# collabora/WhisperLive

Hardware: NVIDIA H100
Metric: audio-sec/sec (RTF^-1) Whisper large-v3, 32 streams, beam 4 (higher is better)
Workload: dtype f16

## Files before the change

### whisperlive_b200/csrc/common.cuh

```cuda
#pragma once
#include <cuda.h>
#include <cuda_fp16.h>
#include <cuda_runtime.h>
#include <stdint.h>
#include <stdio.h>
#include <string.h>
#include <string>
#include <utility>

#define WL_OK 0
#define WL_ERR_CUDA -1
#define WL_ERR_ARG -2
#define WL_ERR_STATE -3
#define WL_ERR_NOMEM -4

namespace wl {

struct Error {
  int code;
  std::string msg;
};

#define WL_CUDA(expr)                                                                         \
  do {                                                                                        \
    cudaError_t _e = (expr);                                                                  \
    if (_e != cudaSuccess) {                                                                  \
      char _b[512];                                                                           \
      snprintf(_b, sizeof(_b), "%s:%d: %s -> %s", __FILE__, __LINE__, #expr, cudaGetErrorString(_e)); \
      throw wl::Error{WL_ERR_CUDA, _b};                                                       \
    }                                                                                         \
  } while (0)

#define WL_CHECK(cond, code, ...)                                  \
  do {                                                             \
    if (!(cond)) {                                                 \
      char _b[512];                                                \
      snprintf(_b, sizeof(_b), __VA_ARGS__);                       \
      throw wl::Error{code, std::string(_b)};                      \
    }                                                              \
  } while (0)

static inline int cdiv(long a, long b) { return (int)((a + b - 1) / b); }
void note_launch(int n);

bool pdl_active();
struct PdlScope {
  explicit PdlScope(bool on);
  ~PdlScope();
  bool prev;
};

#ifdef __CUDACC__
template <typename... KArgs, typename... Args>
static inline void launch_kernel(void (*kernel)(KArgs...), dim3 grid, dim3 block, size_t smem, cudaStream_t st, Args&&... args) {
  cudaLaunchConfig_t cfg;
  memset(&cfg, 0, sizeof(cfg));
  cfg.gridDim = grid;
  cfg.blockDim = block;
  cfg.dynamicSmemBytes = smem;
  cfg.stream = st;
  cudaLaunchAttribute attr[1];
  attr[0].id = cudaLaunchAttributeProgrammaticStreamSerialization;
  attr[0].val.programmaticStreamSerializationAllowed = 1;
  cfg.attrs = attr;
  cfg.numAttrs = pdl_active() ? 1 : 0;
  WL_CUDA(cudaLaunchKernelEx(&cfg, kernel, KArgs(std::forward<Args>(args))...));
}

constexpr unsigned TL_CAP = 1u << 20;
static __device__ unsigned long long* wl_tl_buf = nullptr;
#ifndef WLB200_TL
#define WLB200_TL 0
#endif
__device__ __forceinline__ void tl_stamp_any(int kernel_id, int what) {
  if (!WLB200_TL) return;
  unsigned long long* buf = wl_tl_buf;
  if (buf != nullptr) {
    unsigned long long t;
    asm volatile("mov.u64 %0, %%globaltimer;" : "=l"(t));
    const unsigned idx = atomicAdd(reinterpret_cast<unsigned*>(buf), 1u);
    if (idx < TL_CAP) buf[1 + idx] = (t << 8) | ((unsigned long long)kernel_id << 2) | (unsigned long long)what;
  }
}
__device__ __forceinline__ void tl_stamp(int kernel_id, int what) {
  if (blockIdx.x == 0 && blockIdx.y == 0 && threadIdx.x == 0) tl_stamp_any(kernel_id, what);
}
static inline void tl_bind_tu(unsigned long long* p) { cudaMemcpyToSymbol(wl_tl_buf, &p, sizeof(p)); }
enum TlKernel : int { TL_EMBED = 1, TL_LN = 2, TL_GEMM_PART = 3, TL_SELF = 4, TL_CROSS = 5, TL_COMBINE = 6, TL_GELU = 7,
                      TL_SROWS = 8, TL_SSTREAMS = 9, TL_GEMM = 10, TL_DSTEP = 11 };

__device__ __forceinline__ uint32_t smem_u32(const void* p) { return (uint32_t)__cvta_generic_to_shared(p); }
__device__ __forceinline__ int lane_id() { return threadIdx.x & 31; }

__device__ __forceinline__ bool elect_one() {
  uint32_t pred;
  asm volatile(
      "{\n\t.reg .pred p;\n\t.reg .b32 r;\n\t"
      "elect.sync r|p, 0xffffffff;\n\t"
      "selp.u32 %0, 1, 0, p;\n\t}"
      : "=r"(pred));
  return pred != 0;
}

__device__ __forceinline__ float gelu_erf(float x) {
  const float ax = fabsf(x);
  float t, e;
  asm("rcp.approx.ftz.f32 %0, %1;" : "=f"(t) : "f"(fmaf(0.3275911f * 0.70710678118654752440f, ax, 1.0f)));
  const float w = ax * 0.84932180028801904272f;
  asm("ex2.approx.ftz.f32 %0, %1;" : "=f"(e) : "f"(-w * w));
  float poly = fmaf(0.5f * 1.061405429f, t, 0.5f * -1.453152027f);
  poly = fmaf(poly, t, 0.5f * 1.421413741f);
  poly = fmaf(poly, t, 0.5f * -0.284496736f);
  poly = fmaf(poly, t, 0.5f * 0.254829592f);
  return fmaxf(x, 0.f) - ax * (poly * t * e);
}

__device__ __forceinline__ void pdl_wait() { asm volatile("griddepcontrol.wait;" ::: "memory"); }
__device__ __forceinline__ void pdl_trigger() { asm volatile("griddepcontrol.launch_dependents;" ::: "memory"); }

__device__ __forceinline__ void named_bar_sync(int id, int n) { asm volatile("bar.sync %0, %1;" ::"r"(id), "r"(n) : "memory"); }
__device__ __forceinline__ void named_bar_arrive(int id, int n) { asm volatile("bar.arrive %0, %1;" ::"r"(id), "r"(n) : "memory"); }

template <int R>
__device__ __forceinline__ void setmaxnreg_dec() { asm volatile("setmaxnreg.dec.sync.aligned.u32 %0;" ::"n"(R)); }
template <int R>
__device__ __forceinline__ void setmaxnreg_inc() { asm volatile("setmaxnreg.inc.sync.aligned.u32 %0;" ::"n"(R)); }

__device__ __forceinline__ float warp_sum(float v) {
#pragma unroll
  for (int o = 16; o > 0; o >>= 1) v += __shfl_xor_sync(0xffffffffu, v, o);
  return v;
}
__device__ __forceinline__ float warp_max(float v) {
#pragma unroll
  for (int o = 16; o > 0; o >>= 1) v = fmaxf(v, __shfl_xor_sync(0xffffffffu, v, o));
  return v;
}

__device__ __forceinline__ void mbar_init(uint64_t* bar, uint32_t count) {
  asm volatile("mbarrier.init.shared::cta.b64 [%0], %1;" ::"r"(smem_u32(bar)), "r"(count));
}
__device__ __forceinline__ void mbar_fence_init() { asm volatile("fence.mbarrier_init.release.cluster;" ::: "memory"); }
__device__ __forceinline__ void mbar_expect_tx(uint64_t* bar, uint32_t bytes) {
  asm volatile("mbarrier.arrive.expect_tx.shared::cta.b64 _, [%0], %1;" ::"r"(smem_u32(bar)), "r"(bytes) : "memory");
}
__device__ __forceinline__ void mbar_arrive(uint64_t* bar) {
  asm volatile("mbarrier.arrive.shared::cta.b64 _, [%0];" ::"r"(smem_u32(bar)) : "memory");
}
__device__ __forceinline__ void mbar_wait(uint64_t* bar, uint32_t parity) {
  asm volatile(
      "{\n\t.reg .pred p;\n\t"
      "WAIT_%=:\n\t"
      "mbarrier.try_wait.parity.shared::cta.b64 p, [%0], %1;\n\t"
      "@p bra DONE_%=;\n\t"
      "bra WAIT_%=;\n\t"
      "DONE_%=:\n\t}" ::"r"(smem_u32(bar)),
      "r"(parity)
      : "memory");
}
__device__ __forceinline__ void fence_proxy_async() { asm volatile("fence.proxy.async.shared::cta;" ::: "memory"); }

__device__ __forceinline__ void tma_prefetch_desc(const void* tmap) {
  asm volatile("prefetch.tensormap [%0];" ::"l"(tmap) : "memory");
}
__device__ __forceinline__ void tma_load_4d(void* dst, const void* tmap, uint64_t* bar, int c0, int c1, int c2, int c3) {
  asm volatile(
      "cp.async.bulk.tensor.4d.shared::cluster.global.tile.mbarrier::complete_tx::bytes [%0], [%1, {%3, %4, %5, %6}], [%2];" ::
          "r"(smem_u32(dst)),
      "l"(tmap), "r"(smem_u32(bar)), "r"(c0), "r"(c1), "r"(c2), "r"(c3)
      : "memory");
}
__device__ __forceinline__ void bulk_load_1d(void* dst, const void* src, uint32_t bytes, uint64_t* bar) {
  asm volatile("cp.async.bulk.shared::cluster.global.mbarrier::complete_tx::bytes [%0], [%1], %2, [%3];" ::"r"(
                   smem_u32(dst)),
               "l"(src), "r"(bytes), "r"(smem_u32(bar))
               : "memory");
}

__device__ __forceinline__ void wgmma_fence() { asm volatile("wgmma.fence.sync.aligned;" ::: "memory"); }
__device__ __forceinline__ void wgmma_commit() { asm volatile("wgmma.commit_group.sync.aligned;" ::: "memory"); }
template <int N>
__device__ __forceinline__ void wgmma_wait() { asm volatile("wgmma.wait_group.sync.aligned %0;" ::"n"(N) : "memory"); }
template <int R>
__device__ __forceinline__ void wgmma_fence_regs(float (&d)[R]) {
#pragma unroll
  for (int i = 0; i < R; ++i) asm volatile("" : "+f"(d[i])::"memory");
}

template <int N>
__device__ __forceinline__ void wgmma_ss(float (&d)[N / 2], uint64_t da, uint64_t db, uint32_t scale_d);
template <>
__device__ __forceinline__ void wgmma_ss<16>(float (&d)[8], uint64_t da, uint64_t db, uint32_t scale_d) {
  asm volatile(
      "{\n\t.reg .pred p;\n\tsetp.ne.b32 p, %10, 0;\n\t"
      "wgmma.mma_async.sync.aligned.m64n16k16.f32.f16.f16 {"
      "%0, %1, %2, %3, %4, %5, %6, %7"
      "}, %8, %9, p, 1, 1, 0, 0;\n\t}"
      : "+f"(d[0]), "+f"(d[1]), "+f"(d[2]), "+f"(d[3]), "+f"(d[4]), "+f"(d[5]), "+f"(d[6]), "+f"(d[7])
      : "l"(da), "l"(db), "r"(scale_d));
}

template <>
__device__ __forceinline__ void wgmma_ss<32>(float (&d)[16], uint64_t da, uint64_t db, uint32_t scale_d) {
  asm volatile(
      "{\n\t.reg .pred p;\n\tsetp.ne.b32 p, %18, 0;\n\t"
      "wgmma.mma_async.sync.aligned.m64n32k16.f32.f16.f16 {"
      "%0, %1, %2, %3, %4, %5, %6, %7, %8, %9, %10, %11, %12, %13, %14, %15"
      "}, %16, %17, p, 1, 1, 0, 0;\n\t}"
      : "+f"(d[0]), "+f"(d[1]), "+f"(d[2]), "+f"(d[3]), "+f"(d[4]), "+f"(d[5]), "+f"(d[6]), "+f"(d[7]),
        "+f"(d[8]), "+f"(d[9]), "+f"(d[10]), "+f"(d[11]), "+f"(d[12]), "+f"(d[13]), "+f"(d[14]), "+f"(d[15])
      : "l"(da), "l"(db), "r"(scale_d));
}

template <>
__device__ __forceinline__ void wgmma_ss<64>(float (&d)[32], uint64_t da, uint64_t db, uint32_t scale_d) {
  asm volatile(
      "{\n\t.reg .pred p;\n\tsetp.ne.b32 p, %34, 0;\n\t"
      "wgmma.mma_async.sync.aligned.m64n64k16.f32.f16.f16 {"
      "%0, %1, %2, %3, %4, %5, %6, %7, %8, %9, %10, %11, %12, %13, %14, %15,"
      "%16, %17, %18, %19, %20, %21, %22, %23, %24, %25, %26, %27, %28, %29, %30, %31"
      "}, %32, %33, p, 1, 1, 0, 0;\n\t}"
      : "+f"(d[0]), "+f"(d[1]), "+f"(d[2]), "+f"(d[3]), "+f"(d[4]), "+f"(d[5]), "+f"(d[6]), "+f"(d[7]),
        "+f"(d[8]), "+f"(d[9]), "+f"(d[10]), "+f"(d[11]), "+f"(d[12]), "+f"(d[13]), "+f"(d[14]), "+f"(d[15]),
        "+f"(d[16]), "+f"(d[17]), "+f"(d[18]), "+f"(d[19]), "+f"(d[20]), "+f"(d[21]), "+f"(d[22]), "+f"(d[23]),
        "+f"(d[24]), "+f"(d[25]), "+f"(d[26]), "+f"(d[27]), "+f"(d[28]), "+f"(d[29]), "+f"(d[30]), "+f"(d[31])
      : "l"(da), "l"(db), "r"(scale_d));
}

template <>
__device__ __forceinline__ void wgmma_ss<128>(float (&d)[64], uint64_t da, uint64_t db, uint32_t scale_d) {
  asm volatile(
      "{\n\t.reg .pred p;\n\tsetp.ne.b32 p, %66, 0;\n\t"
      "wgmma.mma_async.sync.aligned.m64n128k16.f32.f16.f16 {"
      "%0, %1, %2, %3, %4, %5, %6, %7, %8, %9, %10, %11, %12, %13, %14, %15,"
      "%16, %17, %18, %19, %20, %21, %22, %23, %24, %25, %26, %27, %28, %29, %30, %31,"
      "%32, %33, %34, %35, %36, %37, %38, %39, %40, %41, %42, %43, %44, %45, %46, %47,"
      "%48, %49, %50, %51, %52, %53, %54, %55, %56, %57, %58, %59, %60, %61, %62, %63"
      "}, %64, %65, p, 1, 1, 0, 0;\n\t}"
      : "+f"(d[0]), "+f"(d[1]), "+f"(d[2]), "+f"(d[3]), "+f"(d[4]), "+f"(d[5]), "+f"(d[6]), "+f"(d[7]),
        "+f"(d[8]), "+f"(d[9]), "+f"(d[10]), "+f"(d[11]), "+f"(d[12]), "+f"(d[13]), "+f"(d[14]), "+f"(d[15]),
        "+f"(d[16]), "+f"(d[17]), "+f"(d[18]), "+f"(d[19]), "+f"(d[20]), "+f"(d[21]), "+f"(d[22]), "+f"(d[23]),
        "+f"(d[24]), "+f"(d[25]), "+f"(d[26]), "+f"(d[27]), "+f"(d[28]), "+f"(d[29]), "+f"(d[30]), "+f"(d[31]),
        "+f"(d[32]), "+f"(d[33]), "+f"(d[34]), "+f"(d[35]), "+f"(d[36]), "+f"(d[37]), "+f"(d[38]), "+f"(d[39]),
        "+f"(d[40]), "+f"(d[41]), "+f"(d[42]), "+f"(d[43]), "+f"(d[44]), "+f"(d[45]), "+f"(d[46]), "+f"(d[47]),
        "+f"(d[48]), "+f"(d[49]), "+f"(d[50]), "+f"(d[51]), "+f"(d[52]), "+f"(d[53]), "+f"(d[54]), "+f"(d[55]),
        "+f"(d[56]), "+f"(d[57]), "+f"(d[58]), "+f"(d[59]), "+f"(d[60]), "+f"(d[61]), "+f"(d[62]), "+f"(d[63])
      : "l"(da), "l"(db), "r"(scale_d));
}

__device__ __forceinline__ void wgmma_rs_n64(float (&d)[32], const uint32_t (&a)[4], uint64_t db, uint32_t scale_d) {
  asm volatile(
      "{\n\t.reg .pred p;\n\tsetp.ne.b32 p, %37, 0;\n\t"
      "wgmma.mma_async.sync.aligned.m64n64k16.f32.f16.f16 {"
      "%0, %1, %2, %3, %4, %5, %6, %7, %8, %9, %10, %11, %12, %13, %14, %15,"
      "%16, %17, %18, %19, %20, %21, %22, %23, %24, %25, %26, %27, %28, %29, %30, %31"
      "}, {%32, %33, %34, %35}, %36, p, 1, 1, 0;\n\t}"
      : "+f"(d[0]), "+f"(d[1]), "+f"(d[2]), "+f"(d[3]), "+f"(d[4]), "+f"(d[5]), "+f"(d[6]), "+f"(d[7]),
        "+f"(d[8]), "+f"(d[9]), "+f"(d[10]), "+f"(d[11]), "+f"(d[12]), "+f"(d[13]), "+f"(d[14]), "+f"(d[15]),
        "+f"(d[16]), "+f"(d[17]), "+f"(d[18]), "+f"(d[19]), "+f"(d[20]), "+f"(d[21]), "+f"(d[22]), "+f"(d[23]),
        "+f"(d[24]), "+f"(d[25]), "+f"(d[26]), "+f"(d[27]), "+f"(d[28]), "+f"(d[29]), "+f"(d[30]), "+f"(d[31])
      : "r"(a[0]), "r"(a[1]), "r"(a[2]), "r"(a[3]), "l"(db), "r"(scale_d));
}

__device__ __forceinline__ uint64_t wgmma_desc_sw128(uint32_t smem_addr) {
  uint64_t d = 0;
  d |= (uint64_t)((smem_addr & 0x3FFFFu) >> 4);
  d |= (uint64_t)1 << 16;
  d |= (uint64_t)(1024 >> 4) << 32;
  d |= (uint64_t)1 << 62;
  return d;
}

template <int BN>
__device__ __forceinline__ void wgmma_tile_k64(float (&acc)[BN / 2], const uint8_t* sa, const uint8_t* sb, int wg, bool accumulate) {
  const uint64_t adesc = wgmma_desc_sw128(smem_u32(sa + wg * 64 * 128));
  const uint64_t bdesc = wgmma_desc_sw128(smem_u32(sb));
#pragma unroll
  for (int k = 0; k < 4; ++k) wgmma_ss<BN>(acc, adesc + (uint64_t)(2 * k), bdesc + (uint64_t)(2 * k), (accumulate || k > 0) ? 1u : 0u);
}

template <int R, class F>
__device__ __forceinline__ void wgmma_acc_foreach(const float (&d)[R], F&& f) {
  const int l = threadIdx.x & 31, w = (threadIdx.x >> 5) & 3;
  const int r0 = 16 * w + (l >> 2), c0 = 2 * (l & 3);
#pragma unroll
  for (int c = 0; c < R / 4; ++c)
#pragma unroll
    for (int i = 0; i < 2; ++i)
#pragma unroll
      for (int j = 0; j < 2; ++j) f(r0 + 8 * i, 8 * c + c0 + j, d[4 * c + 2 * i + j]);
}
#endif

}
```

### whisperlive_b200/csrc/gemm.cu

```cuda
#include "gemm.cuh"

#include <algorithm>
#include <atomic>
#include <cstdlib>
#include <cstring>
#include <map>
#include <mutex>
#include <vector>

namespace wl {

static std::atomic<long> g_gemm_launches{0};
long gemm_launch_count() { return g_gemm_launches.load(); }

struct GemmKParams {
  int M, N, K;
  int zn1;
  int a_batched, b_batched;
  int a_pos[3], b_pos[3];
  GemmEpilogue e;
  int vec_ok;
  int nz;
  int n_fastest;
};

constexpr int BM = 128;
constexpr int BK = 64;
constexpr int A_STAGE_BYTES = BM * BK * 2;

enum EpiKind : int { EPI_ROW = 0, EPI_COL = 1, EPI_HEADSPLIT = 2 };

template <int cnt, int KIND>
__device__ __forceinline__ void epilogue_chunk(const GemmKParams& p, long m, int n0, const uint32_t (&v)[cnt], int i1, int i2) {
  const GemmEpilogue& e = p.e;
  if (m >= p.M) return;
  if constexpr (KIND == EPI_HEADSPLIT && cnt >= 8) {
    const int mi = (int)m;
    const int b = mi / e.hs_S, s = mi % e.hs_S;
    const int h = n0 >> 6, dd = n0 & 63;
    const long slot = e.hs_slots[b];
    float x[cnt];
#pragma unroll
    for (int i = 0; i < cnt; ++i) x[i] = __uint_as_float(v[i]);
    if (e.bias) {
#pragma unroll
      for (int i = 0; i < cnt; i += 8) {
        if (n0 + i >= p.N) break;
#pragma unroll
        for (int j = 0; j < 8; ++j) x[i + j] += e.bias[n0 + i + j];
      }
    }
    __half* dst = (__half*)e.out + slot * e.hs_slot_stride + ((long)h * e.hs_S + s) * 64;
#pragma unroll
    for (int i = 0; i < cnt; i += 8) {
      if (n0 + i >= p.N) break;
      __align__(16) __half2 h2[4];
#pragma unroll
      for (int j = 0; j < 4; ++j) h2[j] = __floats2half2_rn(x[i + 2 * j], x[i + 2 * j + 1]);
      *reinterpret_cast<uint4*>(dst + ((((dd + i) >> 3) ^ (s & 7)) << 3)) = *reinterpret_cast<const uint4*>(h2);
    }
    return;
  }
  const long obase = (long)i1 * e.ob1 + (long)i2 * e.ob2 + m * e.ldm;
  const long rbase = (long)i1 * e.rb1 + (long)i2 * e.rb2 + m * e.rldm;
  const float bm = (e.bias && e.bias_on_m) ? e.bias[m] : 0.f;
  if constexpr (KIND == EPI_ROW && cnt >= 8) {
    if (n0 + cnt <= p.N) {
      float x[cnt];
#pragma unroll
      for (int i = 0; i < cnt; ++i) x[i] = __uint_as_float(v[i]) + bm;
      if (e.bias && !e.bias_on_m) {
#pragma unroll
        for (int i = 0; i < cnt; i += 4) {
          const float4 b4 = *reinterpret_cast<const float4*>(e.bias + n0 + i);
          x[i] += b4.x; x[i + 1] += b4.y; x[i + 2] += b4.z; x[i + 3] += b4.w;
        }
      }
      if (e.gelu) {
#pragma unroll
        for (int i = 0; i < cnt; ++i) x[i] = gelu_erf(x[i]);
      }
      if (e.resid) {
        const float* r = e.resid + rbase + n0;
        float4 r4[cnt / 4];
#pragma unroll
        for (int i = 0; i < cnt / 4; ++i) r4[i] = *reinterpret_cast<const float4*>(r + 4 * i);
#pragma unroll
        for (int i = 0; i < cnt / 4; ++i) {
          x[4 * i] += r4[i].x; x[4 * i + 1] += r4[i].y; x[4 * i + 2] += r4[i].z; x[4 * i + 3] += r4[i].w;
        }
      }
#pragma unroll
      for (int i = 0; i < cnt; i += 8) {
        if (e.out_f32) {
          float* o = (float*)e.out + obase + n0 + i;
          *reinterpret_cast<float4*>(o) = make_float4(x[i], x[i + 1], x[i + 2], x[i + 3]);
          *reinterpret_cast<float4*>(o + 4) = make_float4(x[i + 4], x[i + 5], x[i + 6], x[i + 7]);
        } else {
          __align__(16) __half2 h2[4];
#pragma unroll
          for (int j = 0; j < 4; ++j) h2[j] = __floats2half2_rn(x[i + 2 * j], x[i + 2 * j + 1]);
          *reinterpret_cast<uint4*>((__half*)e.out + obase + n0 + i) = *reinterpret_cast<const uint4*>(h2);
        }
      }
      return;
    }
#pragma unroll
    for (int i = 0; i < cnt; i += 8) {
      const int n = n0 + i;
      if (n >= p.N) break;
      if (n + 8 > p.N) {
#pragma unroll
        for (int j = 0; j < 8; ++j) {
          if (n + j < p.N) {
            float x1 = __uint_as_float(v[i + j]) + bm;
            if (e.bias && !e.bias_on_m) x1 += e.bias[n + j];
            if (e.gelu) x1 = gelu_erf(x1);
            if (e.resid) x1 += e.resid[rbase + n + j];
            if (e.out_f32) ((float*)e.out)[obase + n + j] = x1;
            else ((__half*)e.out)[obase + n + j] = __float2half_rn(x1);
          }
        }
        continue;
      }
      float x[8];
#pragma unroll
      for (int j = 0; j < 8; ++j) x[j] = __uint_as_float(v[i + j]) + bm;
      if (e.bias && !e.bias_on_m) {
        const float4 b0 = *reinterpret_cast<const float4*>(e.bias + n), b1 = *reinterpret_cast<const float4*>(e.bias + n + 4);
        x[0] += b0.x; x[1] += b0.y; x[2] += b0.z; x[3] += b0.w;
        x[4] += b1.x; x[5] += b1.y; x[6] += b1.z; x[7] += b1.w;
      }
      if (e.gelu) {
#pragma unroll
        for (int j = 0; j < 8; ++j) x[j] = gelu_erf(x[j]);
      }
      if (e.resid) {
        const float* r = e.resid + rbase + n;
        const float4 r0 = *reinterpret_cast<const float4*>(r), r1 = *reinterpret_cast<const float4*>(r + 4);
        x[0] += r0.x; x[1] += r0.y; x[2] += r0.z; x[3] += r0.w;
        x[4] += r1.x; x[5] += r1.y; x[6] += r1.z; x[7] += r1.w;
      }
      if (e.out_f32) {
        float* o = (float*)e.out + obase + n;
        *reinterpret_cast<float4*>(o) = make_float4(x[0], x[1], x[2], x[3]);
        *reinterpret_cast<float4*>(o + 4) = make_float4(x[4], x[5], x[6], x[7]);
      } else {
        __align__(16) __half2 h2[4];
#pragma unroll
        for (int j = 0; j < 4; ++j) h2[j] = __floats2half2_rn(x[2 * j], x[2 * j + 1]);
        *reinterpret_cast<uint4*>((__half*)e.out + obase + n) = *reinterpret_cast<const uint4*>(h2);
      }
    }
    return;
  }
  if constexpr (KIND == EPI_COL || cnt < 8) {
#pragma unroll
  for (int i = 0; i < cnt; ++i) {
    const int n = n0 + i;
    if (n >= p.N) break;
    float x = __uint_as_float(v[i]) + bm;
    if (e.bias && !e.bias_on_m) x += e.bias[n];
    if (e.gelu) x = gelu_erf(x);
    if (e.resid) x += e.resid[rbase + (long)n * e.rldn];
    const long o = obase + (long)n * e.ldn;
    if (e.out_f32) ((float*)e.out)[o] = x;
    else ((__half*)e.out)[o] = __float2half_rn(x);
  }
  }
}

__device__ __forceinline__ void tile_decode(const GemmKParams& p, int t, int tiles_m, int tiles_n, int& tile_m, int& tile_n, int& zz) {
  if (p.n_fastest) {
    tile_n = t % tiles_n;
    const int r = t / tiles_n;
    tile_m = r % tiles_m;
    zz = r / tiles_m;
  } else {
    tile_m = t % tiles_m;
    const int r = t / tiles_m;
    tile_n = r % tiles_n;
    zz = r / tiles_n;
  }
}

template <int BN>
struct EpiStage {
  static constexpr int CH = BN < 64 ? BN : 64;
  static constexpr int LD = CH + 4;
  static constexpr int BYTES = 2 * 64 * LD * 4;
};
template <int BN, int STAGES>
__host__ __device__ constexpr int gemm_smem_bytes() { return STAGES * (A_STAGE_BYTES + BN * BK * 2) + EpiStage<BN>::BYTES + 1024 + 512; }

struct TileCoord {
  int tile_m, tile_n, i1, i2;
};
__device__ __forceinline__ TileCoord tile_coord(const GemmKParams& p, int t, int tiles_m, int tiles_n) {
  TileCoord c;
  int z;
  tile_decode(p, t, tiles_m, tiles_n, c.tile_m, c.tile_n, z);
  c.i1 = z % p.zn1;
  c.i2 = z / p.zn1;
  return c;
}

template <int BN, int STAGES>
__device__ __forceinline__ void gemm_produce(const CUtensorMap* tmA, const CUtensorMap* tmB, const GemmKParams& p, uint8_t* sA,
                                             uint8_t* sB, uint64_t* full, uint64_t* empty, int tiles_m, int tiles_n,
                                             int total_tiles, int total_kb) {
  constexpr int B_STAGE_BYTES = BN * BK * 2;
  int stage = 0;
  uint32_t phase = 0;
  bool first = true;
  auto slot = [](const int (&pos)[3], int s, int row, int j1, int j2) {
    return pos[0] == s ? row : (pos[1] == s ? j1 : (pos[2] == s ? j2 : 0));
  };
  for (int t = blockIdx.x; t < total_tiles; t += gridDim.x) {
    const TileCoord tc = tile_coord(p, t, tiles_m, tiles_n);
    const int a1 = p.a_batched ? tc.i1 : 0, a2 = p.a_batched ? tc.i2 : 0;
    const int b1 = p.b_batched ? tc.i1 : 0, b2 = p.b_batched ? tc.i2 : 0;
    const int ca1 = slot(p.a_pos, 1, tc.tile_m * BM, a1, a2), ca2 = slot(p.a_pos, 2, tc.tile_m * BM, a1, a2),
              ca3 = slot(p.a_pos, 3, tc.tile_m * BM, a1, a2);
    const int cb1 = slot(p.b_pos, 1, tc.tile_n * BN, b1, b2), cb2 = slot(p.b_pos, 2, tc.tile_n * BN, b1, b2),
              cb3 = slot(p.b_pos, 3, tc.tile_n * BN, b1, b2);
    if (first) {
      if (blockIdx.x == 0) tl_stamp_any(TL_GEMM, 0);
      pdl_wait();
      if (blockIdx.x == 0) tl_stamp_any(TL_GEMM, 1);
      first = false;
    }
    for (int kb = 0; kb < total_kb; ++kb) {
      const int k0 = kb * BK;
      mbar_wait(&empty[stage], phase ^ 1);
      mbar_expect_tx(&full[stage], A_STAGE_BYTES + B_STAGE_BYTES);
      tma_load_4d(sA + stage * A_STAGE_BYTES, tmA, &full[stage], k0, ca1, ca2, ca3);
      tma_load_4d(sB + stage * B_STAGE_BYTES, tmB, &full[stage], k0, cb1, cb2, cb3);
      if (++stage == STAGES) { stage = 0; phase ^= 1; }
    }
  }
}

template <int BN, int KIND>
__device__ __forceinline__ void epilogue_rows64(const GemmKParams& p, const float (&acc)[BN / 2], float* stg, int bar_id, long m0,
                                                int n0, int i1, int i2) {
  using ES = EpiStage<BN>;
  const int tw = threadIdx.x & 127;
  const int row = tw & 63, half = tw >> 6;
#pragma unroll
  for (int ch = 0; ch < BN / ES::CH; ++ch) {
    wgmma_acc_foreach(acc, [&](int r, int c, float v) {
      if (c >= ch * ES::CH && c < (ch + 1) * ES::CH) stg[r * ES::LD + c - ch * ES::CH] = v;
    });
    named_bar_sync(bar_id, 128);
    constexpr int CNT = ES::CH / 2;
    uint32_t v[CNT];
    const float4* src = reinterpret_cast<const float4*>(stg + row * ES::LD + half * CNT);
#pragma unroll
    for (int i = 0; i < CNT / 4; ++i) {
      const float4 q = src[i];
      v[4 * i] = __float_as_uint(q.x); v[4 * i + 1] = __float_as_uint(q.y);
      v[4 * i + 2] = __float_as_uint(q.z); v[4 * i + 3] = __float_as_uint(q.w);
    }
    named_bar_sync(bar_id, 128);
    epilogue_chunk<CNT, KIND>(p, m0 + row, n0 + ch * ES::CH + half * CNT, v, i1, i2);
  }
}

template <int BN, int STAGES, int MIN_CTAS, int KIND>
__global__ void __launch_bounds__(384, MIN_CTAS)
gemm_tn_kernel(const __grid_constant__ CUtensorMap tmA, const __grid_constant__ CUtensorMap tmB,
               const __grid_constant__ GemmKParams p) {
  extern __shared__ uint8_t smem_raw[];
  uint8_t* base = smem_raw + ((1024u - (smem_u32(smem_raw) & 1023u)) & 1023u);
  constexpr int B_STAGE_BYTES = BN * BK * 2;
  using ES = EpiStage<BN>;
  uint8_t* sA = base;
  uint8_t* sB = base + STAGES * A_STAGE_BYTES;
  float* stg_all = reinterpret_cast<float*>(sB + STAGES * B_STAGE_BYTES);
  uint64_t* full = reinterpret_cast<uint64_t*>(reinterpret_cast<uint8_t*>(stg_all) + ES::BYTES);
  uint64_t* empty = full + STAGES;

  const int warp = threadIdx.x >> 5;
  const int tiles_m = (p.M + BM - 1) / BM, tiles_n = (p.N + BN - 1) / BN;
  const int total_tiles = tiles_m * tiles_n * p.nz;
  const int total_kb = (p.K + BK - 1) / BK;
  pdl_trigger();

  if (warp == 0 && elect_one()) {
    tma_prefetch_desc(&tmA);
    tma_prefetch_desc(&tmB);
  }
  if (warp == 1 && elect_one()) {
    for (int s = 0; s < STAGES; ++s) {
      mbar_init(&full[s], 1);
      mbar_init(&empty[s], 8);
    }
    mbar_fence_init();
  }
  __syncthreads();

  if (warp == 0) {
    if (elect_one()) gemm_produce<BN, STAGES>(&tmA, &tmB, p, sA, sB, full, empty, tiles_m, tiles_n, total_tiles, total_kb);
  } else if (warp >= 4) {
    const int wg = (warp >> 2) - 1;
    float* stg = stg_all + wg * 64 * ES::LD;
    int stage = 0;
    uint32_t phase = 0;
    pdl_wait();
    for (int t = blockIdx.x; t < total_tiles; t += gridDim.x) {
      const TileCoord tc = tile_coord(p, t, tiles_m, tiles_n);
      float acc[BN / 2];
#pragma unroll
      for (int i = 0; i < BN / 2; ++i) acc[i] = 0.f;
      int prev = -1;
      for (int kb = 0; kb < total_kb; ++kb) {
        mbar_wait(&full[stage], phase);
        wgmma_fence();
        wgmma_tile_k64<BN>(acc, sA + stage * A_STAGE_BYTES, sB + stage * B_STAGE_BYTES, wg, kb > 0);
        wgmma_commit();
        wgmma_wait<1>();
        if (prev >= 0 && lane_id() == 0) mbar_arrive(&empty[prev]);
        prev = stage;
        if (++stage == STAGES) { stage = 0; phase ^= 1; }
      }
      wgmma_wait<0>();
      wgmma_fence_regs(acc);
      if (prev >= 0 && lane_id() == 0) mbar_arrive(&empty[prev]);
      epilogue_rows64<BN, KIND>(p, acc, stg, 1 + wg, (long)tc.tile_m * BM + wg * 64, tc.tile_n * BN, tc.i1, tc.i2);
    }
  }
}

constexpr int PP_STAGES = 5;
constexpr int PP_BAR = 4;
constexpr int PP_PRODUCER_REGS = 40, PP_CONSUMER_REGS = 232;

template <int KIND>
__global__ void __launch_bounds__(384, 1)
gemm_pingpong_kernel(const __grid_constant__ CUtensorMap tmA, const __grid_constant__ CUtensorMap tmB,
                     const __grid_constant__ GemmKParams p) {
  constexpr int BN = 128, STAGES = PP_STAGES;
  extern __shared__ uint8_t smem_raw[];
  uint8_t* base = smem_raw + ((1024u - (smem_u32(smem_raw) & 1023u)) & 1023u);
  constexpr int B_STAGE_BYTES = BN * BK * 2;
  using ES = EpiStage<BN>;
  uint8_t* sA = base;
  uint8_t* sB = base + STAGES * A_STAGE_BYTES;
  float* stg_all = reinterpret_cast<float*>(sB + STAGES * B_STAGE_BYTES);
  uint64_t* full = reinterpret_cast<uint64_t*>(reinterpret_cast<uint8_t*>(stg_all) + ES::BYTES);
  uint64_t* empty = full + STAGES;

  const int warp = threadIdx.x >> 5;
  const int tiles_m = (p.M + BM - 1) / BM, tiles_n = (p.N + BN - 1) / BN;
  const int total_tiles = tiles_m * tiles_n * p.nz;
  const int total_kb = (p.K + BK - 1) / BK;
  pdl_trigger();

  if (warp == 0 && elect_one()) {
    tma_prefetch_desc(&tmA);
    tma_prefetch_desc(&tmB);
  }
  if (warp == 1 && elect_one()) {
    for (int s = 0; s < STAGES; ++s) {
      mbar_init(&full[s], 1);
      mbar_init(&empty[s], 4);
    }
    mbar_fence_init();
  }
  __syncthreads();

  if (warp < 4) {
    setmaxnreg_dec<PP_PRODUCER_REGS>();
    if (warp == 0 && elect_one())
      gemm_produce<BN, STAGES>(&tmA, &tmB, p, sA, sB, full, empty, tiles_m, tiles_n, total_tiles, total_kb);
    return;
  }
  setmaxnreg_inc<PP_CONSUMER_REGS>();
  const int wg = (warp >> 2) - 1;
  float* stg = stg_all + wg * 64 * ES::LD;
  pdl_wait();
  if (wg == 1) named_bar_arrive(PP_BAR, 256);
  for (int j = wg, t = blockIdx.x + wg * gridDim.x; t < total_tiles; j += 2, t += 2 * gridDim.x) {
    const TileCoord tc = tile_coord(p, t, tiles_m, tiles_n);
    const long it0 = (long)j * total_kb;
    int stage = (int)(it0 % STAGES);
    uint32_t phase = (uint32_t)((it0 / STAGES) & 1);
    float acc[2][BN / 2];
#pragma unroll
    for (int h = 0; h < 2; ++h)
#pragma unroll
      for (int i = 0; i < BN / 2; ++i) acc[h][i] = 0.f;
    named_bar_sync(PP_BAR + wg, 256);
    int prev = -1;
    for (int kb = 0; kb < total_kb; ++kb) {
      mbar_wait(&full[stage], phase);
      wgmma_fence();
      wgmma_tile_k64<BN>(acc[0], sA + stage * A_STAGE_BYTES, sB + stage * B_STAGE_BYTES, 0, kb > 0);
      wgmma_tile_k64<BN>(acc[1], sA + stage * A_STAGE_BYTES, sB + stage * B_STAGE_BYTES, 1, kb > 0);
      wgmma_commit();
      wgmma_wait<1>();
      if (prev >= 0 && lane_id() == 0) mbar_arrive(&empty[prev]);
      prev = stage;
      if (++stage == STAGES) { stage = 0; phase ^= 1; }
    }
    if (t + gridDim.x < total_tiles) named_bar_arrive(PP_BAR + (wg ^ 1), 256);
    wgmma_wait<0>();
    wgmma_fence_regs(acc[0]);
    wgmma_fence_regs(acc[1]);
    if (prev >= 0 && lane_id() == 0) mbar_arrive(&empty[prev]);
#pragma unroll
    for (int h = 0; h < 2; ++h)
      epilogue_rows64<BN, KIND>(p, acc[h], stg, 1 + wg, (long)tc.tile_m * BM + h * 64, tc.tile_n * BN, tc.i1, tc.i2);
  }
}

typedef CUresult (*EncodeTiledFn)(CUtensorMap*, CUtensorMapDataType, cuuint32_t, void*, const cuuint64_t*,
                                  const cuuint64_t*, const cuuint32_t*, const cuuint32_t*, CUtensorMapInterleave,
                                  CUtensorMapSwizzle, CUtensorMapL2promotion, CUtensorMapFloatOOBfill);

static EncodeTiledFn encode_fn() {
  static EncodeTiledFn fn = nullptr;
  static std::once_flag once;
  std::call_once(once, [] {
    void* p = nullptr;
    cudaDriverEntryPointQueryResult q;
    cudaError_t e = cudaGetDriverEntryPoint("cuTensorMapEncodeTiled", &p, cudaEnableDefault, &q);
    if (e == cudaSuccess && q == cudaDriverEntryPointSuccess) fn = (EncodeTiledFn)p;
  });
  WL_CHECK(fn != nullptr, WL_ERR_CUDA, "cuTensorMapEncodeTiled is not available from the driver");
  return fn;
}

struct TmapKey {
  const void* ptr;
  long rows, k, ld, s1, s2;
  int n1, n2, box_rows, box_k;
  bool operator<(const TmapKey& o) const { return memcmp(this, &o, sizeof(TmapKey)) < 0; }
};

static TmapInfo get_tmap(const GemmOperand& op, int box_rows, int box_k = BK);
TmapInfo make_tmap(const GemmOperand& op, int box_rows, int box_k) { return get_tmap(op, box_rows, box_k); }

static TmapInfo get_tmap(const GemmOperand& op, int box_rows, int box_k) {
  static std::map<TmapKey, TmapInfo> cache;
  static std::mutex mu;
  TmapKey key;
  memset(&key, 0, sizeof(key));
  key.ptr = op.ptr; key.rows = op.rows; key.k = op.k; key.ld = op.ld; key.s1 = op.s1; key.s2 = op.s2;
  key.n1 = op.n1; key.n2 = op.n2; key.box_rows = box_rows; key.box_k = box_k;
  std::lock_guard<std::mutex> lk(mu);
  auto it = cache.find(key);
  if (it != cache.end()) return it->second;
  WL_CHECK(((uintptr_t)op.ptr & 15) == 0, WL_ERR_ARG, "GEMM operand pointer must be 16-byte aligned");
  struct D { long size, stride; int role; };
  std::vector<D> real, single;
  const D all[3] = {{op.rows, op.ld, 0}, {op.n1, op.s1, 1}, {op.n2, op.s2, 2}};
  for (const D& d : all) ((d.role == 0 || d.size > 1) ? real : single).push_back(d);
  std::stable_sort(real.begin(), real.end(), [](const D& x, const D& y) { return x.stride < y.stride; });
  std::vector<D> order = real;
  for (D d : single) {
    d.stride = order.back().stride * order.back().size;
    order.push_back(d);
  }
  TmapInfo info;
  cuuint64_t dims[4] = {(cuuint64_t)op.k, 1, 1, 1};
  cuuint64_t strides[3];
  cuuint32_t box[4] = {(cuuint32_t)box_k, 1, 1, 1};
  cuuint32_t estr[4] = {1, 1, 1, 1};
  for (int i = 0; i < 3; ++i) {
    WL_CHECK(order[i].stride > 0 && (order[i].stride * 2) % 16 == 0, WL_ERR_ARG,
             "GEMM operand stride %ld elements (dim role %d) is not a positive multiple of 16 bytes", order[i].stride, order[i].role);
    dims[1 + i] = (cuuint64_t)order[i].size;
    strides[i] = (cuuint64_t)order[i].stride * 2;
    if (order[i].role == 0) box[1 + i] = (cuuint32_t)box_rows;
    info.pos[order[i].role] = 1 + i;
  }
  CUresult r = encode_fn()(&info.tm, CU_TENSOR_MAP_DATA_TYPE_FLOAT16, 4, (void*)op.ptr, dims, strides, box, estr,
                           CU_TENSOR_MAP_INTERLEAVE_NONE, CU_TENSOR_MAP_SWIZZLE_128B, CU_TENSOR_MAP_L2_PROMOTION_L2_256B,
                           CU_TENSOR_MAP_FLOAT_OOB_FILL_NONE);
  WL_CHECK(r == CUDA_SUCCESS, WL_ERR_CUDA,
           "cuTensorMapEncodeTiled failed (%d) dims={%llu,%llu,%llu,%llu} strides={%llu,%llu,%llu} box_rows=%d", (int)r,
           (unsigned long long)dims[0], (unsigned long long)dims[1], (unsigned long long)dims[2], (unsigned long long)dims[3],
           (unsigned long long)strides[0], (unsigned long long)strides[1], (unsigned long long)strides[2], box_rows);
  if (cache.size() > 8192) cache.clear();
  cache.emplace(key, info);
  return info;
}

static int num_sms() {
  static int sms = 0;
  if (!sms) { int dev = 0; cudaGetDevice(&dev); cudaDeviceGetAttribute(&sms, cudaDevAttrMultiProcessorCount, dev); }
  return sms;
}

template <int BN, int STAGES, int MIN_CTAS, int KIND>
static void launch_cfg(cudaStream_t stream, const CUtensorMap& ta, const CUtensorMap& tb, const GemmKParams& p, int Z) {
  constexpr int smem = gemm_smem_bytes<BN, STAGES>();
  GemmKParams q = p;
  q.nz = Z;
  const long tiles = (long)cdiv(p.N, BN) * cdiv(p.M, BM) * Z;
  const int grid = (int)std::min<long>(tiles, (long)num_sms() * MIN_CTAS);
  launch_kernel(gemm_tn_kernel<BN, STAGES, MIN_CTAS, KIND>, dim3(grid), dim3(384), (size_t)smem, stream, ta, tb, q);
  g_gemm_launches++;
}

template <int KIND>
static void launch_pingpong(cudaStream_t stream, const CUtensorMap& ta, const CUtensorMap& tb, const GemmKParams& p, int Z) {
  constexpr int smem = gemm_smem_bytes<128, PP_STAGES>();
  GemmKParams q = p;
  q.nz = Z;
  const long tiles = (long)cdiv(p.N, 128) * cdiv(p.M, BM) * Z;
  const int grid = (int)std::min<long>(tiles, num_sms());
  launch_kernel(gemm_pingpong_kernel<KIND>, dim3(grid), dim3(384), (size_t)smem, stream, ta, tb, q);
  g_gemm_launches++;
}

template <int BN, int STAGES, int MIN_CTAS, int KIND>
static void prime_cfg() {
  constexpr int smem = gemm_smem_bytes<BN, STAGES>();
  WL_CUDA(cudaFuncSetAttribute(gemm_tn_kernel<BN, STAGES, MIN_CTAS, KIND>, cudaFuncAttributeMaxDynamicSharedMemorySize, smem));
}

template <int KIND>
static void prime_kind() {
  prime_cfg<16, 8, 1, KIND>();
  prime_cfg<32, 8, 1, KIND>();
  prime_cfg<64, 6, 1, KIND>();
  prime_cfg<128, 5, 1, KIND>();
}
void gemm_tl_bind(unsigned long long* p) { tl_bind_tu(p); }
template <int KIND>
static void prime_pingpong() {
  constexpr int smem = gemm_smem_bytes<128, PP_STAGES>();
  WL_CUDA(cudaFuncSetAttribute(gemm_pingpong_kernel<KIND>, cudaFuncAttributeMaxDynamicSharedMemorySize, smem));
}
void gemm_prime() {
  prime_kind<EPI_ROW>();
  prime_kind<EPI_COL>();
  prime_kind<EPI_HEADSPLIT>();
  prime_pingpong<EPI_ROW>();
  prime_pingpong<EPI_COL>();
  prime_pingpong<EPI_HEADSPLIT>();
}

template <int KIND>
static void launch_kind(int bn, cudaStream_t stream, const CUtensorMap& ta, const CUtensorMap& tb, const GemmKParams& p, int Z) {
  switch (bn) {
    case 16: launch_cfg<16, 8, 1, KIND>(stream, ta, tb, p, Z); break;
    case 32: launch_cfg<32, 8, 1, KIND>(stream, ta, tb, p, Z); break;
    case 64: launch_cfg<64, 6, 1, KIND>(stream, ta, tb, p, Z); break;
    case 128: launch_cfg<128, 5, 1, KIND>(stream, ta, tb, p, Z); break;
    default: WL_CHECK(false, WL_ERR_ARG, "unsupported BN %d", bn);
  }
}

static int env_int(const char* name, int dflt) {
  const char* v = getenv(name);
  return v ? atoi(v) : dflt;
}

static GemmKParams make_params(const GemmOperand& A, const GemmOperand& B, int M, int N, int K, const GemmEpilogue& epi,
                               int* Z) {
  WL_CHECK(M > 0 && N > 0 && K > 0, WL_ERR_ARG, "gemm_tn: empty problem %dx%dx%d", M, N, K);
  const int za = A.n1 * A.n2, zb = B.n1 * B.n2;
  WL_CHECK(za == 1 || zb == 1 || (A.n1 == B.n1 && A.n2 == B.n2), WL_ERR_ARG, "gemm_tn: batch shapes differ");
  GemmKParams p;
  memset(&p, 0, sizeof(p));
  p.M = M; p.N = N; p.K = K;
  p.a_batched = za > 1; p.b_batched = zb > 1;
  p.zn1 = za > 1 ? A.n1 : B.n1;
  *Z = za > zb ? za : zb;
  p.e = epi;
  p.vec_ok = 0;
  p.n_fastest = (zb == 1 && (long)N * K * 2 <= (24L << 20) && (long)M * K > (long)N * K) ? 1 : 0;
  if (epi.mode == GEMM_STORE && epi.ldn == 1) {
    const int a = epi.out_f32 ? 4 : 8;
    bool ok = ((uintptr_t)epi.out & 15) == 0 && epi.ldm % 8 == 0 && epi.ob1 % 8 == 0 && epi.ob2 % 8 == 0;
    (void)a;
    if (epi.bias && !epi.bias_on_m) ok = ok && ((uintptr_t)epi.bias & 15) == 0;
    if (epi.resid)
      ok = ok && epi.rldn == 1 && ((uintptr_t)epi.resid & 15) == 0 && epi.rldm % 4 == 0 && epi.rb1 % 4 == 0 && epi.rb2 % 4 == 0;
    p.vec_ok = ok ? 1 : 0;
  }
  if (epi.mode == GEMM_HEADSPLIT) {
    WL_CHECK(!epi.out_f32 && !epi.gelu && !epi.resid && !epi.bias_on_m && N % 64 == 0 && epi.hs_slots, WL_ERR_ARG,
             "gemm_tn: bad head-split epilogue");
  }
  return p;
}

static int pick_bn(int N) {
  static const int force_bn = env_int("WLB200_BN", 0);
  if (force_bn) return force_bn;
  if (N <= 16) return 16;
  if (N <= 32) return 32;
  if (N <= 64) return 64;
  return 128;
}

static bool pingpong_pays(int bn, long tiles) { return bn == 128 && tiles >= 2L * num_sms(); }

GemmVariant gemm_tn_variant(int M, int N, int K, int Z) {
  (void)K;
  const int bn = pick_bn(N);
  return pingpong_pays(bn, (long)cdiv(M, BM) * cdiv(N, bn) * Z) ? GEMM_PINGPONG : GEMM_CLASSIC;
}

void gemm_tn(cudaStream_t stream, const GemmOperand& A, const GemmOperand& B, int M, int N, int K, const GemmEpilogue& epi,
             GemmVariant variant) {
  int Z;
  GemmKParams p = make_params(A, B, M, N, K, epi, &Z);
  int bn = pick_bn(N);
  if (epi.mode == GEMM_HEADSPLIT && bn < 64) bn = 64;
  const TmapInfo ia = get_tmap(A, BM), ib = get_tmap(B, bn);
  const CUtensorMap& ta = ia.tm;
  const CUtensorMap& tb = ib.tm;
  for (int i = 0; i < 3; ++i) { p.a_pos[i] = ia.pos[i]; p.b_pos[i] = ib.pos[i]; }
  bool pingpong = pingpong_pays(bn, (long)cdiv(M, BM) * cdiv(N, bn) * Z);
  if (variant != GEMM_AUTO) {
    WL_CHECK(variant == GEMM_CLASSIC || bn == 128, WL_ERR_ARG, "gemm_tn: the ping-pong kernel needs N tiles of 128");
    pingpong = variant == GEMM_PINGPONG;
  }
  if (pingpong) {
    if (epi.mode == GEMM_HEADSPLIT) launch_pingpong<EPI_HEADSPLIT>(stream, ta, tb, p, Z);
    else if (p.vec_ok) launch_pingpong<EPI_ROW>(stream, ta, tb, p, Z);
    else launch_pingpong<EPI_COL>(stream, ta, tb, p, Z);
  } else if (epi.mode == GEMM_HEADSPLIT) launch_kind<EPI_HEADSPLIT>(bn, stream, ta, tb, p, Z);
  else if (p.vec_ok) launch_kind<EPI_ROW>(bn, stream, ta, tb, p, Z);
  else launch_kind<EPI_COL>(bn, stream, ta, tb, p, Z);
}

__global__ void gemm_tn_simt_kernel(GemmOperand A, GemmOperand B, GemmKParams p) {
  const long n = blockIdx.x * (long)blockDim.x + threadIdx.x;
  const long m = blockIdx.y;
  const int z = blockIdx.z;
  if (n >= p.N) return;
  const int i1 = z % p.zn1, i2 = z / p.zn1;
  const __half* a = A.ptr + (p.a_batched ? (long)i1 * A.s1 + (long)i2 * A.s2 : 0) + m * A.ld;
  const __half* b = B.ptr + (p.b_batched ? (long)i1 * B.s1 + (long)i2 * B.s2 : 0) + n * B.ld;
  float acc = 0.f;
  const int ka = (int)(A.k < p.K ? A.k : p.K), kb = (int)(B.k < p.K ? B.k : p.K);
  const int kk = ka < kb ? ka : kb;
  for (int k = 0; k < kk; ++k) acc = fmaf(__half2float(a[k]), __half2float(b[k]), acc);
  uint32_t v[1] = {__float_as_uint(acc)};
  GemmKParams q = p;
  q.vec_ok = 0;
  if (q.e.mode == GEMM_HEADSPLIT) {
    const GemmEpilogue& e = q.e;
    const int bb = (int)(m / e.hs_S), s = (int)(m % e.hs_S);
    float x = acc + (e.bias ? e.bias[n] : 0.f);
    ((__half*)e.out)[(long)e.hs_slots[bb] * e.hs_slot_stride + ((long)(n >> 6) * e.hs_S + s) * 64 + (((((int)n & 63) >> 3) ^ (s & 7)) << 3) + (n & 7)] = __float2half_rn(x);
    return;
  }
  epilogue_chunk<1, EPI_COL>(q, m, (int)n, v, i1, i2);
}

void gemm_tn_simt(cudaStream_t stream, const GemmOperand& A, const GemmOperand& B, int M, int N, int K, const GemmEpilogue& epi) {
  int Z;
  GemmKParams p = make_params(A, B, M, N, K, epi, &Z);
  dim3 grid(cdiv(N, 128), M, Z);
  gemm_tn_simt_kernel<<<grid, 128, 0, stream>>>(A, B, p);
  WL_CUDA(cudaGetLastError());
  g_gemm_launches++;
}

}
```

Measured before the change: 810.7.

## Add 2-CTA cluster TMA multicast to ping-pong GEMM for shared operand tiles

Launches the ping-pong GEMM as 2-CTA clusters in which the two CTAs work on neighbouring tiles that share one operand. Each CTA loads half of the shared A or B tile and multicasts it to both CTAs, and empty-barrier arrivals are sent across the cluster. The aim is to halve global/L2 traffic for the shared operand. In exchange it pads the tile counts to even numbers, adds cluster syncs and cross-CTA barrier coupling, and sizes the grid from the cluster occupancy query.

```diff
diff --git a/whisperlive_b200/csrc/common.cuh b/whisperlive_b200/csrc/common.cuh
--- a/whisperlive_b200/csrc/common.cuh
+++ b/whisperlive_b200/csrc/common.cuh
@@ -121,6 +121,15 @@
 __device__ __forceinline__ void named_bar_sync(int id, int n) { asm volatile("bar.sync %0, %1;" ::"r"(id), "r"(n) : "memory"); }
 __device__ __forceinline__ void named_bar_arrive(int id, int n) { asm volatile("bar.arrive %0, %1;" ::"r"(id), "r"(n) : "memory"); }
 
+__device__ __forceinline__ uint32_t cluster_ctarank() {
+  uint32_t r;
+  asm volatile("mov.u32 %0, %%cluster_ctarank;" : "=r"(r));
+  return r;
+}
+__device__ __forceinline__ void cluster_sync() {
+  asm volatile("barrier.cluster.arrive.release;\n\tbarrier.cluster.wait.acquire;" ::: "memory");
+}
+
 template <int R>
 __device__ __forceinline__ void setmaxnreg_dec() { asm volatile("setmaxnreg.dec.sync.aligned.u32 %0;" ::"n"(R)); }
 template <int R>
@@ -146,6 +155,14 @@
 }
 __device__ __forceinline__ void mbar_arrive(uint64_t* bar) {
   asm volatile("mbarrier.arrive.shared::cta.b64 _, [%0];" ::"r"(smem_u32(bar)) : "memory");
+}
+__device__ __forceinline__ void mbar_arrive_cluster(uint64_t* bar, uint32_t cta) {
+  asm volatile(
+      "{\n\t.reg .b32 ra;\n\t"
+      "mapa.shared::cluster.u32 ra, %0, %1;\n\t"
+      "mbarrier.arrive.shared::cluster.b64 _, [ra];\n\t}" ::"r"(smem_u32(bar)),
+      "r"(cta)
+      : "memory");
 }
 __device__ __forceinline__ void mbar_wait(uint64_t* bar, uint32_t parity) {
   asm volatile(
@@ -168,6 +185,14 @@
       "cp.async.bulk.tensor.4d.shared::cluster.global.tile.mbarrier::complete_tx::bytes [%0], [%1, {%3, %4, %5, %6}], [%2];" ::
           "r"(smem_u32(dst)),
       "l"(tmap), "r"(smem_u32(bar)), "r"(c0), "r"(c1), "r"(c2), "r"(c3)
+      : "memory");
+}
+__device__ __forceinline__ void tma_load_4d_multicast(void* dst, const void* tmap, uint64_t* bar, uint16_t cta_mask, int c0, int c1,
+                                                      int c2, int c3) {
+  asm volatile(
+      "cp.async.bulk.tensor.4d.shared::cluster.global.tile.mbarrier::complete_tx::bytes.multicast::cluster"
+      " [%0], [%1, {%4, %5, %6, %7}], [%2], %3;" ::"r"(smem_u32(dst)),
+      "l"(tmap), "r"(smem_u32(bar)), "h"(cta_mask), "r"(c0), "r"(c1), "r"(c2), "r"(c3)
       : "memory");
 }
 __device__ __forceinline__ void bulk_load_1d(void* dst, const void* src, uint32_t bytes, uint64_t* bar) {
diff --git a/whisperlive_b200/csrc/gemm.cu b/whisperlive_b200/csrc/gemm.cu
--- a/whisperlive_b200/csrc/gemm.cu
+++ b/whisperlive_b200/csrc/gemm.cu
@@ -205,11 +205,13 @@
   return c;
 }
 
-template <int BN, int STAGES>
+template <int BN, int STAGES, bool PAIR = false>
 __device__ __forceinline__ void gemm_produce(const CUtensorMap* tmA, const CUtensorMap* tmB, const GemmKParams& p, uint8_t* sA,
                                              uint8_t* sB, uint64_t* full, uint64_t* empty, int tiles_m, int tiles_n,
-                                             int total_tiles, int total_kb) {
+                                             int total_tiles, int total_kb, uint32_t rank = 0) {
   constexpr int B_STAGE_BYTES = BN * BK * 2;
+  const bool share_a = PAIR && p.n_fastest, share_b = PAIR && !p.n_fastest;
+  const int a_half = share_a ? (int)rank * (BM / 2) : 0, b_half = share_b ? (int)rank * (BN / 2) : 0;
   int stage = 0;
   uint32_t phase = 0;
   bool first = true;
@@ -220,10 +222,9 @@
     const TileCoord tc = tile_coord(p, t, tiles_m, tiles_n);
     const int a1 = p.a_batched ? tc.i1 : 0, a2 = p.a_batched ? tc.i2 : 0;
     const int b1 = p.b_batched ? tc.i1 : 0, b2 = p.b_batched ? tc.i2 : 0;
-    const int ca1 = slot(p.a_pos, 1, tc.tile_m * BM, a1, a2), ca2 = slot(p.a_pos, 2, tc.tile_m * BM, a1, a2),
-              ca3 = slot(p.a_pos, 3, tc.tile_m * BM, a1, a2);
-    const int cb1 = slot(p.b_pos, 1, tc.tile_n * BN, b1, b2), cb2 = slot(p.b_pos, 2, tc.tile_n * BN, b1, b2),
-              cb3 = slot(p.b_pos, 3, tc.tile_n * BN, b1, b2);
+    const int ra = tc.tile_m * BM + a_half, rb = tc.tile_n * BN + b_half;
+    const int ca1 = slot(p.a_pos, 1, ra, a1, a2), ca2 = slot(p.a_pos, 2, ra, a1, a2), ca3 = slot(p.a_pos, 3, ra, a1, a2);
+    const int cb1 = slot(p.b_pos, 1, rb, b1, b2), cb2 = slot(p.b_pos, 2, rb, b1, b2), cb3 = slot(p.b_pos, 3, rb, b1, b2);
     if (first) {
       if (blockIdx.x == 0) tl_stamp_any(TL_GEMM, 0);
       pdl_wait();
@@ -234,8 +235,14 @@
       const int k0 = kb * BK;
       mbar_wait(&empty[stage], phase ^ 1);
       mbar_expect_tx(&full[stage], A_STAGE_BYTES + B_STAGE_BYTES);
-      tma_load_4d(sA + stage * A_STAGE_BYTES, tmA, &full[stage], k0, ca1, ca2, ca3);
-      tma_load_4d(sB + stage * B_STAGE_BYTES, tmB, &full[stage], k0, cb1, cb2, cb3);
+      if (share_a)
+        tma_load_4d_multicast(sA + stage * A_STAGE_BYTES + a_half * 128, tmA, &full[stage], 3, k0, ca1, ca2, ca3);
+      else
+        tma_load_4d(sA + stage * A_STAGE_BYTES, tmA, &full[stage], k0, ca1, ca2, ca3);
+      if (share_b)
+        tma_load_4d_multicast(sB + stage * B_STAGE_BYTES + b_half * 128, tmB, &full[stage], 3, k0, cb1, cb2, cb3);
+      else
+        tma_load_4d(sB + stage * B_STAGE_BYTES, tmB, &full[stage], k0, cb1, cb2, cb3);
       if (++stage == STAGES) { stage = 0; phase ^= 1; }
     }
   }
@@ -335,9 +342,17 @@
 constexpr int PP_STAGES = 5;
 constexpr int PP_BAR = 4;
 constexpr int PP_PRODUCER_REGS = 40, PP_CONSUMER_REGS = 232;
+constexpr int PP_CLUSTER = 2;
+
+__host__ __device__ __forceinline__ void pingpong_tiles(int M, int N, int n_fastest, int& tiles_m, int& tiles_n) {
+  tiles_m = (M + BM - 1) / BM;
+  tiles_n = (N + 127) / 128;
+  if (n_fastest) tiles_n += tiles_n & 1;
+  else tiles_m += tiles_m & 1;
+}
 
 template <int KIND>
-__global__ void __launch_bounds__(384, 1)
+__global__ void __cluster_dims__(PP_CLUSTER, 1, 1) __launch_bounds__(384, 1)
 gemm_pingpong_kernel(const __grid_constant__ CUtensorMap tmA, const __grid_constant__ CUtensorMap tmB,
                      const __grid_constant__ GemmKParams p) {
   constexpr int BN = 128, STAGES = PP_STAGES;
@@ -352,7 +367,9 @@
   uint64_t* empty = full + STAGES;
 
   const int warp = threadIdx.x >> 5;
-  const int tiles_m = (p.M + BM - 1) / BM, tiles_n = (p.N + BN - 1) / BN;
+  const uint32_t rank = cluster_ctarank();
+  int tiles_m, tiles_n;
+  pingpong_tiles(p.M, p.N, p.n_fastest, tiles_m, tiles_n);
   const int total_tiles = tiles_m * tiles_n * p.nz;
   const int total_kb = (p.K + BK - 1) / BK;
   pdl_trigger();
@@ -364,55 +381,56 @@
   if (warp == 1 && elect_one()) {
     for (int s = 0; s < STAGES; ++s) {
       mbar_init(&full[s], 1);
-      mbar_init(&empty[s], 4);
+      mbar_init(&empty[s], 4 * PP_CLUSTER);
     }
     mbar_fence_init();
   }
-  __syncthreads();
+  cluster_sync();
 
   if (warp < 4) {
     setmaxnreg_dec<PP_PRODUCER_REGS>();
     if (warp == 0 && elect_one())
-      gemm_produce<BN, STAGES>(&tmA, &tmB, p, sA, sB, full, empty, tiles_m, tiles_n, total_tiles, total_kb);
-    return;
-  }
-  setmaxnreg_inc<PP_CONSUMER_REGS>();
-  const int wg = (warp >> 2) - 1;
-  float* stg = stg_all + wg * 64 * ES::LD;
-  pdl_wait();
-  if (wg == 1) named_bar_arrive(PP_BAR, 256);
-  for (int j = wg, t = blockIdx.x + wg * gridDim.x; t < total_tiles; j += 2, t += 2 * gridDim.x) {
-    const TileCoord tc = tile_coord(p, t, tiles_m, tiles_n);
-    const long it0 = (long)j * total_kb;
-    int stage = (int)(it0 % STAGES);
-    uint32_t phase = (uint32_t)((it0 / STAGES) & 1);
-    float acc[2][BN / 2];
-#pragma unroll
-    for (int h = 0; h < 2; ++h)
-#pragma unroll
-      for (int i = 0; i < BN / 2; ++i) acc[h][i] = 0.f;
-    named_bar_sync(PP_BAR + wg, 256);
-    int prev = -1;
-    for (int kb = 0; kb < total_kb; ++kb) {
-      mbar_wait(&full[stage], phase);
-      wgmma_fence();
-      wgmma_tile_k64<BN>(acc[0], sA + stage * A_STAGE_BYTES, sB + stage * B_STAGE_BYTES, 0, kb > 0);
-      wgmma_tile_k64<BN>(acc[1], sA + stage * A_STAGE_BYTES, sB + stage * B_STAGE_BYTES, 1, kb > 0);
-      wgmma_commit();
-      wgmma_wait<1>();
-      if (prev >= 0 && lane_id() == 0) mbar_arrive(&empty[prev]);
-      prev = stage;
-      if (++stage == STAGES) { stage = 0; phase ^= 1; }
-    }
-    if (t + gridDim.x < total_tiles) named_bar_arrive(PP_BAR + (wg ^ 1), 256);
-    wgmma_wait<0>();
-    wgmma_fence_regs(acc[0]);
-    wgmma_fence_regs(acc[1]);
-    if (prev >= 0 && lane_id() == 0) mbar_arrive(&empty[prev]);
-#pragma unroll
-    for (int h = 0; h < 2; ++h)
-      epilogue_rows64<BN, KIND>(p, acc[h], stg, 1 + wg, (long)tc.tile_m * BM + h * 64, tc.tile_n * BN, tc.i1, tc.i2);
-  }
+      gemm_produce<BN, STAGES, true>(&tmA, &tmB, p, sA, sB, full, empty, tiles_m, tiles_n, total_tiles, total_kb, rank);
+  } else {
+    setmaxnreg_inc<PP_CONSUMER_REGS>();
+    const int wg = (warp >> 2) - 1;
+    float* stg = stg_all + wg * 64 * ES::LD;
+    pdl_wait();
+    if (wg == 1) named_bar_arrive(PP_BAR, 256);
+    for (int j = wg, t = blockIdx.x + wg * gridDim.x; t < total_tiles; j += 2, t += 2 * gridDim.x) {
+      const TileCoord tc = tile_coord(p, t, tiles_m, tiles_n);
+      const long it0 = (long)j * total_kb;
+      int stage = (int)(it0 % STAGES);
+      uint32_t phase = (uint32_t)((it0 / STAGES) & 1);
+      float acc[2][BN / 2];
+#pragma unroll
+      for (int h = 0; h < 2; ++h)
+#pragma unroll
+        for (int i = 0; i < BN / 2; ++i) acc[h][i] = 0.f;
+      named_bar_sync(PP_BAR + wg, 256);
+      int prev = -1;
+      for (int kb = 0; kb < total_kb; ++kb) {
+        mbar_wait(&full[stage], phase);
+        wgmma_fence();
+        wgmma_tile_k64<BN>(acc[0], sA + stage * A_STAGE_BYTES, sB + stage * B_STAGE_BYTES, 0, kb > 0);
+        wgmma_tile_k64<BN>(acc[1], sA + stage * A_STAGE_BYTES, sB + stage * B_STAGE_BYTES, 1, kb > 0);
+        wgmma_commit();
+        wgmma_wait<1>();
+        if (prev >= 0 && lane_id() < 2) mbar_arrive_cluster(&empty[prev], rank ^ lane_id());
+        prev = stage;
+        if (++stage == STAGES) { stage = 0; phase ^= 1; }
+      }
+      if (t + gridDim.x < total_tiles) named_bar_arrive(PP_BAR + (wg ^ 1), 256);
+      wgmma_wait<0>();
+      wgmma_fence_regs(acc[0]);
+      wgmma_fence_regs(acc[1]);
+      if (prev >= 0 && lane_id() < 2) mbar_arrive_cluster(&empty[prev], rank ^ lane_id());
+#pragma unroll
+      for (int h = 0; h < 2; ++h)
+        epilogue_rows64<BN, KIND>(p, acc[h], stg, 1 + wg, (long)tc.tile_m * BM + h * 64, tc.tile_n * BN, tc.i1, tc.i2);
+    }
+  }
+  cluster_sync();
 }
 
 typedef CUresult (*EncodeTiledFn)(CUtensorMap*, CUtensorMapDataType, cuuint32_t, void*, const cuuint64_t*,
@@ -505,13 +523,18 @@
   g_gemm_launches++;
 }
 
+static int g_pp_clusters = 0;
+
 template <int KIND>
 static void launch_pingpong(cudaStream_t stream, const CUtensorMap& ta, const CUtensorMap& tb, const GemmKParams& p, int Z) {
   constexpr int smem = gemm_smem_bytes<128, PP_STAGES>();
   GemmKParams q = p;
   q.nz = Z;
-  const long tiles = (long)cdiv(p.N, 128) * cdiv(p.M, BM) * Z;
-  const int grid = (int)std::min<long>(tiles, num_sms());
+  int tiles_m, tiles_n;
+  pingpong_tiles(p.M, p.N, p.n_fastest, tiles_m, tiles_n);
+  const long tiles = (long)tiles_m * tiles_n * Z;
+  const int grid = (int)std::min<long>(tiles, (long)PP_CLUSTER * g_pp_clusters);
+  WL_CHECK(grid > 0 && grid % PP_CLUSTER == 0, WL_ERR_STATE, "gemm_tn: ping-pong grid %d (gemm_prime not run?)", grid);
   launch_kernel(gemm_pingpong_kernel<KIND>, dim3(grid), dim3(384), (size_t)smem, stream, ta, tb, q);
   g_gemm_launches++;
 }
@@ -534,6 +557,15 @@
 static void prime_pingpong() {
   constexpr int smem = gemm_smem_bytes<128, PP_STAGES>();
   WL_CUDA(cudaFuncSetAttribute(gemm_pingpong_kernel<KIND>, cudaFuncAttributeMaxDynamicSharedMemorySize, smem));
+  cudaLaunchConfig_t cfg;
+  memset(&cfg, 0, sizeof(cfg));
+  cfg.gridDim = dim3(PP_CLUSTER * num_sms());
+  cfg.blockDim = dim3(384);
+  cfg.dynamicSmemBytes = smem;
+  int clusters = 0;
+  WL_CUDA(cudaOccupancyMaxActiveClusters(&clusters, gemm_pingpong_kernel<KIND>, &cfg));
+  WL_CHECK(clusters > 0, WL_ERR_CUDA, "gemm_pingpong_kernel: no 2-CTA cluster fits on this device");
+  g_pp_clusters = g_pp_clusters ? std::min(g_pp_clusters, clusters) : clusters;
 }
 void gemm_prime() {
   prime_kind<EPI_ROW>();
@@ -613,15 +645,16 @@
   GemmKParams p = make_params(A, B, M, N, K, epi, &Z);
   int bn = pick_bn(N);
   if (epi.mode == GEMM_HEADSPLIT && bn < 64) bn = 64;
-  const TmapInfo ia = get_tmap(A, BM), ib = get_tmap(B, bn);
-  const CUtensorMap& ta = ia.tm;
-  const CUtensorMap& tb = ib.tm;
-  for (int i = 0; i < 3; ++i) { p.a_pos[i] = ia.pos[i]; p.b_pos[i] = ib.pos[i]; }
   bool pingpong = pingpong_pays(bn, (long)cdiv(M, BM) * cdiv(N, bn) * Z);
   if (variant != GEMM_AUTO) {
     WL_CHECK(variant == GEMM_CLASSIC || bn == 128, WL_ERR_ARG, "gemm_tn: the ping-pong kernel needs N tiles of 128");
     pingpong = variant == GEMM_PINGPONG;
   }
+  const bool half_a = pingpong && p.n_fastest, half_b = pingpong && !p.n_fastest;
+  const TmapInfo ia = get_tmap(A, half_a ? BM / 2 : BM), ib = get_tmap(B, half_b ? bn / 2 : bn);
+  const CUtensorMap& ta = ia.tm;
+  const CUtensorMap& tb = ib.tm;
+  for (int i = 0; i < 3; ++i) { p.a_pos[i] = ia.pos[i]; p.b_pos[i] = ib.pos[i]; }
   if (pingpong) {
     if (epi.mode == GEMM_HEADSPLIT) launch_pingpong<EPI_HEADSPLIT>(stream, ta, tb, p, Z);
     else if (p.vec_ok) launch_pingpong<EPI_ROW>(stream, ta, tb, p, Z);
```

Measured after the change: 820.9, median of 6. +1.3%, better.
